# wsakobe/CylinderTag

Measured on AMD Instinct MI355X. Metric: frames/sec detect() 1920x1080, higher is better.
Workload: dtype u8; 1 GPU; synthetic 1920x1080 random-stripe frames, 4096 per step over 1 GPU(s), 4 planted CTag_2f12c markers each, detect(img,5,true,5), inputs resident in HBM; frames_per_gpu=4096, chunk=4096, parallelism=frames sharded, dp1, gather=none (1 GPU)

## Files before the change

cylindertag_amd/csrc/k_quad.hip:

```cpp
#include "ctag_internal.h"
#include "ctag_math.h"
#include <cstdio>
#include <type_traits>
#include <cstdlib>

namespace ctag {

struct QuadPtrs {
    const uint16_t* labels;
    const int32_t* tile_base;
    const int32_t* root_of;
    const int32_t* ncand;
    const Candidate* cand;
    QuadOut* quads;
    uint32_t* frame_flags;
    int32_t* line_count;
    int32_t* clp_used;
    uint32_t* cl_pool;
    LineDesc* line_desc;
    int32_t* line_sorted;
    int32_t* line_long;
    float* line_fit;
    CandAux* cand_aux;
    const uint8_t* pick_table;
// ... 38 lines not shown
__device__ __forceinline__ bool solve2x2(float a00, float a01, float a10, float a11, float b0, float b1, float& x0, float& x1) {
    double d = (double)a00 * a11 - (double)a01 * a10;
    if (d == 0.) return false;
    d = 1. / d;
    const float t = (float)(((double)b0 * a11 - (double)b1 * a01) * d);
    x1 = (float)(((double)b1 * a00 - (double)b0 * a10) * d);
    x0 = t;
    return true;
}

struct CvRng {
    uint64_t state;
    __device__ unsigned next() {
        state = (uint64_t)(unsigned)state * 4164903690U + (unsigned)(state >> 32);
        return (unsigned)state;
    }
};

#ifndef CTAG_WCAP
#define CTAG_WCAP 16
#endif
#ifndef CTAG_WUNROLL
#define CTAG_WUNROLL 2
#endif
#define CTAG_PRAGMA_(x) _Pragma(#x)
#define CTAG_PRAGMA(x) CTAG_PRAGMA_(x)
constexpr int kWCap = CTAG_WCAP;
struct GlobalPts {
    const uint32_t* p;
    __device__ __forceinline__ float2 operator()(int j) const {
        const uint32_t v = p[j];
        return make_float2((float)ux(v), (float)uy(v));
    }
};
struct LdsPts {
    const float2* p;
    __device__ __forceinline__ float2 operator()(int j) const { return p[j]; }
};
struct LdsPackedPts {
    const uint32_t* p;
    __device__ __forceinline__ float2 operator()(int j) const {
        const uint32_t v = p[j];
        return make_float2((float)ux(v), (float)uy(v));
    }
};
struct TablePicks {
    const uint8_t* t;
    __device__ __forceinline__ int operator()(int i) const { return t[i]; }
};
struct ListPicks {
    const uint16_t* t;
    __device__ __forceinline__ int operator()(int i) const { return t[i]; }
};
struct AllPicks {
    __device__ __forceinline__ int operator()(int i) const { return i; }
};
struct RestartResult {
    float line[4];
    double err;
};
__device__ __forceinline__ RestartResult restart_result(const float* res, int rstride) {
    RestartResult r;
    for (int q = 0; q < 4; q++) r.line[q] = res[q * rstride];
    const uint64_t lo = ctm::f32_to_bits(res[4 * rstride]), hi = ctm::f32_to_bits(res[5 * rstride]);
    r.err = ctm::bits_to_f64(lo | (hi << 32));
    return r;
}
template <class Pts, class Picks>
__device__ __forceinline__ void welsch_first_fit(const Pts pts, const Picks picks, int npick, float* line) {
    double x = 0, y = 0, x2 = 0, y2 = 0, xy = 0, w = 0;
    for (int i = 0; i < npick; i++) {
        const float2 p = pts(picks(i));
        const float px = p.x, py = p.y;
        x += px;
        y += py;
        x2 += px * px;
        y2 += py * py;
        xy += px * py;
        w += 1.f;
    }
    moments_to_line(x, y, x2, y2, xy, w, line);
}
template <int WS, class Pts>
__device__ __forceinline__ bool welsch_rounds(const Pts pts, int n, double EPS, float* line, double& err, int it0, int it_stop, bool resume, float* wc, int ncache) {
    float prev[4] = {0.f, 0.f, 0.f, 0.f};
    const float c = 1 / 2.9846f;
#ifdef CTAG_WELSCH_MINERR_IN_LOOP
    double berr = 1.7976931348623157e308;
    float bl[4] = {0.f, 0.f, 0.f, 0.f};
#define CTAG_WELSCH_HAND_ON()       \
    do {                            \
        for (int q = 0; q < 4; q++) line[q] = bl[q]; \
        err = berr;                 \
    } while (0)
#else
#define CTAG_WELSCH_HAND_ON() do { } while (0)
#endif
    for (int it = it0; it < 30; it++) {
        if (it > 0 && !(resume && it == it0)) {
            const float t = line[0] * prev[0] + line[1] * prev[1];
            if (t >= ctm::kAcosBelowTenMilli) {
                const float dx = ctm::fabs32(line[2] - prev[2]);
                const float dy = ctm::fabs32(line[3] - prev[3]);
                const float d = dx > dy ? dx : dy;
                if (d < 0.01f) {
                    CTAG_WELSCH_HAND_ON();
                    return true;
                }
            }
        }
        if (it == it_stop) return false;
        const float lx = line[2], ly = line[3], nx = line[1], ny = -line[0];
        double sum_w = 0;
        err = 0;
        float2 pn0 = pts(min(0, n - 1));
        CTAG_PRAGMA(unroll CTAG_WUNROLL)
        for (int j = 0; j < ncache; j++) {
            const float2 p = pn0;
            pn0 = pts(j + 1);
            const float x = p.x - lx, y = p.y - ly;
            const float r = ctm::fabs32(nx * x + ny * y);
            err += r;
            const float wj = ctm::exp32_nonpos(-r * r * c * c);
            wc[j * WS] = wj;
            sum_w += wj;
        }
        float2 pn1 = pts(min(ncache, n - 1));
        CTAG_PRAGMA(unroll CTAG_WUNROLL)
        for (int j = ncache; j < n; j++) {
            const float2 p = pn1;
            pn1 = pts(j + 1);
            const float x = p.x - lx, y = p.y - ly;
            const float r = ctm::fabs32(nx * x + ny * y);
            err += r;
            sum_w += ctm::exp32_nonpos(-r * r * c * c);
        }
#ifdef CTAG_WELSCH_MINERR_IN_LOOP
        if (err < berr) {
            berr = err;
            for (int q = 0; q < 4; q++) bl[q] = line[q];
            if (err < EPS) return true;
        }
#else
        if (err < EPS) return true;
#endif
        double x = 0, y = 0, x2 = 0, y2 = 0, xy = 0, w = 0;
        if (ctm::fabs64(sum_w) > 1.1920928955078125e-07) {
            const double inv = 1. / sum_w;
            float2 pn2 = pts(min(0, n - 1));
            CTAG_PRAGMA(unroll CTAG_WUNROLL)
            for (int j = 0; j < ncache; j++) {
                const float2 p = pn2;
                pn2 = pts(j + 1);
                const float px = p.x, py = p.y;
                const float wj = (float)(wc[j * WS] * inv);
                x += wj * px;
                y += wj * py;
                x2 += wj * px * px;
                y2 += wj * py * py;
                xy += wj * px * py;
                w += wj;
            }
            float2 pn3 = pts(min(ncache, n - 1));
            CTAG_PRAGMA(unroll CTAG_WUNROLL)
            for (int j = ncache; j < n; j++) {
                const float2 p = pn3;
                pn3 = pts(j + 1);
                const float px = p.x, py = p.y;
                const float r = ctm::fabs32(nx * (px - lx) + ny * (py - ly));
                const float wj = (float)(ctm::exp32_nonpos(-r * r * c * c) * inv);
                x += wj * px;
                y += wj * py;
                x2 += wj * px * px;
                y2 += wj * py * py;
                xy += wj * px * py;
                w += wj;
            }
        } else {
            float2 pn4 = pts(min(0, n - 1));
            for (int j = 0; j < n; j++) {
                const float2 p = pn4;
                pn4 = pts(j + 1);
                const float px = p.x, py = p.y;
                x += px;
                y += py;
                x2 += px * px;
                y2 += py * py;
                xy += px * py;
                w += 1.f;
            }
        }
        prev[0] = line[0];
        prev[1] = line[1];
        prev[2] = line[2];
        prev[3] = line[3];
        moments_to_line(x, y, x2, y2, xy, w, line);
    }
    CTAG_WELSCH_HAND_ON();
    return true;
}
#undef CTAG_WELSCH_HAND_ON
__device__ __forceinline__ void restart_store(float* res, int rstride, const float* line, double err) {
    for (int q = 0; q < 4; q++) res[q * rstride] = line[q];
    const uint64_t eb = ctm::f64_to_bits(err);
    res[4 * rstride] = ctm::bits_to_f32((uint32_t)eb);
    res[5 * rstride] = ctm::bits_to_f32((uint32_t)(eb >> 32));
}
template <int WS, class Pts, class Picks>
__device__ __forceinline__ void welsch_restart(const Pts pts, int n, const Picks picks, int npick, double EPS, float* res, int rstride, float* wc) {
    float line[4];
    double err = 0;
    welsch_first_fit(pts, picks, npick, line);
    (void)welsch_rounds<WS>(pts, n, EPS, line, err, 0, 30, false, wc, min(n, kWCap));
    restart_store(res, rstride, line, err);
}

#ifndef CTAG_PACK_WORDS
#define CTAG_PACK_WORDS 5120
#endif
#ifndef CTAG_PACK_WAVES
#define CTAG_PACK_WAVES 2
#endif
constexpr int kPackWords = CTAG_PACK_WORDS;
#ifndef CTAG_PACK_WAVES_P2
#define CTAG_PACK_WAVES_P2 4
#endif
constexpr int kPackWordsSmall = 2560, kPackWavesSmall = 4, kPackWavesSmallP2 = CTAG_PACK_WAVES_P2;
constexpr int kUnwind = 8;
constexpr int kWaveWords = 8192;
constexpr int kWaveWordsMax = 36864;
__host__ __device__ __forceinline__ int pack_points(int w, int h) { return min(2 * (w + h), w * h) + 1; }
__host__ __device__ __forceinline__ int pack_need(int w, int h) {
    const int C = pack_points(w, h);
    return ((w + 1) & ~1) + 2 * h + 2 * C + 4;
}
constexpr int kScanWords = 2048;
__host__ __device__ __forceinline__ int scan_need(int w, int h) { return w + 3 * h + 4; }
constexpr int kMaskScanWords = 512, kMaskScanWordsLarge = 2048;
// ... 1520 lines not shown
                else
                    sg_expand_line<SG>(W, n, init, end, sl, lane0, sgshift, k_thr_expand, (float)(g.hcols > g.hrows ? g.hcols : g.hrows), REFPRM ? 3.0e-6f : P.expand_eps, nl, nr);
                rdp_mark(2);
                const int m = end - init + 1 + nl + nr;
                const int a = ((init - nl) % n + n) % n;
                const int b = (end + nr) % n;
                const bool wrap = a > b;
                const int span0 = wrap ? n - 1 : b;
                const int keep = tri2(span0) <= k_c2_near ? 1 : 0;
                const int offc = cl_off[cnt_b];
                for (int k = sl; k < m; k += SG) {
                    int idx;
                    if (!wrap) {
                        idx = b - k;
                    } else {
                        idx = (k < n - a) ? (n - 1 - k) : (b - (k - (n - a)));
                    }
                    if (offc + k < C + 64) CLg[offc + k] = W[idx];
                }
                const int new_n = n - m + keep;
                if (!wrap) {
                    for (int k = sl; k < new_n; k += SG) {
                        int src;
                        if (k < a) src = k;
                        else if (keep && k == a) src = b;
                        else src = k - keep + m;
                        Wn[k] = W[src];
                    }
                } else {
                    const int mid = a - b - 1;
                    for (int k = sl; k < new_n; k += SG) Wn[k] = (k < mid) ? W[b + 1 + k] : W[n - 1];
                }
                SG_SYNC();
                const int back = wrap ? 0 : a;
                cl_off[cnt_b + 1] = min(offc + m, C + 64);
                cnt_b++;
                init = (back >= new_n) ? 0 : back;
                n = new_n;
                uint32_t* t = W;
                W = Wn;
                Wn = t;
                rdp_mark(3);
                break;
            }
        }
        if (SG == 64 && P.stamps && lane == 0)
        {
            for (int q = 0; q < 4; q++) atomicAdd(&P.stamps[16 + q], rdp_acc[q]);
            for (int q = 0; q < 3; q++) atomicAdd(&P.stamps[20 + q], exp_dbg[q]);
        }
        stamp(3);
        bool ok = true;
        for (int j = 0; j < 4; j++) {
            const int len = (j < cnt_b) ? (cl_off[j + 1] - cl_off[j]) : 0;
            if (len < 2) ok = false;
        }
        if (cl_off[min(cnt_b, 4)] >= C + 64) ok = false;
        int l0 = -1;
        if (ok) {
            if (sl == 0) l0 = atomicAdd(&P.line_count[frame], 4);
            l0 = __shfl(l0, lane0);
            if (l0 + 4 > P.line_cap) {
                ok = false;
                if (sl == 0) atomicOr(&P.frame_flags[frame], CTAG_FLAG_POOL_OVERFLOW);
            }
        }
        if (ok && sl < 4) {
            LineDesc d;
            d.off = (uint32_t)(p0 + cl_off[sl]);
            d.n = cl_off[sl + 1] - cl_off[sl];
            P.line_desc[(size_t)frame * P.line_cap + l0 + sl] = d;
        }
        if (sl == 0) {
            aux->line0 = ok ? l0 : -1;
            aux->acx = ok ? acx : 0.f;
            aux->acy = ok ? acy : 0.f;
            aux->n_boundary = n_boundary;
        }
        stamp(4);
    }
}

constexpr int kWShort = 10;
constexpr int kLineSortThreads = 1024;
__global__ __launch_bounds__(kLineSortThreads) void k_line_sort(QuadPtrs P, int nframes) {
    __shared__ int s_n[kLdsLines];
    __shared__ int s_long;
    const int frame = blockIdx.x;
    if (frame >= nframes) return;
    const int L = min(P.line_count[frame], P.line_cap);
    const LineDesc* d = P.line_desc + (size_t)frame * P.line_cap;
    int32_t* out = P.line_sorted + (size_t)frame * P.line_cap;
    if (threadIdx.x == 0) s_long = 0;
    __syncthreads();
    if (L > kLdsLines) {
        constexpr int kB = 2048;
        static_assert(kB - 1 > kLatPoints && kB + 1 <= kLdsLines, "shared bucket");
        auto bucket_of = [&](int n) { return kB - 1 - min(n, kB - 1); };
        for (int b = threadIdx.x; b <= kB; b += kLineSortThreads) s_n[b] = 0;
        __syncthreads();
        int mine = 0;
        for (int i = threadIdx.x; i < L; i += kLineSortThreads) {
            const int n = d[i].n;
            atomicAdd(&s_n[bucket_of(n)], 1);
            mine += n > kWShort ? 1 : 0;
        }
        if (mine) atomicAdd(&s_long, mine);
        __syncthreads();
        if (threadIdx.x == 0) {
            P.line_long[frame] = s_long;
            int run = 0;
            for (int b = 0; b < kB; b++) {
                const int v = s_n[b];
                s_n[b] = run;
                run += v;
            }
        }
        __syncthreads();
        for (int i = threadIdx.x; i < L; i += kLineSortThreads) out[atomicAdd(&s_n[bucket_of(d[i].n)], 1)] = i;
        return;
    }
    int mine = 0;
    for (int i = threadIdx.x; i < L; i += kLineSortThreads) {
        const int n = d[i].n;
        s_n[i] = n;
        mine += n > kWShort ? 1 : 0;
    }
    if (mine) atomicAdd(&s_long, mine);
    __syncthreads();
    if (threadIdx.x == 0) P.line_long[frame] = s_long;
    for (int i = threadIdx.x; i < L; i += kLineSortThreads) {
        const int ni = s_n[i];
        int rank = 0;
        for (int j = 0; j < L; j++) {
            const int nj = s_n[j];
            rank += (nj > ni || (nj == ni && j < i)) ? 1 : 0;
        }
        out[rank] = i;
    }
}

__device__ __forceinline__ void welsch_select(const QuadPtrs& P, int frame, int lid, int n, const float* res, int kstride, int rstride, int count) {
    const double EPS = n * 1.1920928955078125e-07;
    double min_err = 1.7976931348623157e308;
    float best[4] = {0.f, 0.f, 0.f, 0.f};
    for (int kk = 0; kk < count; kk++) {
        const RestartResult r = restart_result(res + kk * kstride, rstride);
        if (r.err < min_err) {
            min_err = r.err;
            for (int q = 0; q < 4; q++) best[q] = r.line[q];
#ifndef CTAG_WELSCH_MINERR_IN_LOOP
            if (r.err < EPS) break;
#endif
        }
    }
    float* o = P.line_fit + ((size_t)frame * P.line_cap + lid) * 4;
    for (int q = 0; q < 4; q++) o[q] = best[q];
}

#ifndef CTAG_WELSCH_BLOCK_WAVES
#define CTAG_WELSCH_BLOCK_WAVES 4
#endif
constexpr int kWB = CTAG_WELSCH_BLOCK_WAVES;
constexpr int kWT = kWB * 64;
constexpr int kWE = kWT / 20;
constexpr int kWRes = 10;
#ifdef CTAG_WELSCH_MINERR_IN_LOOP
#undef CTAG_WELSCH_REGROUP_AT
#define CTAG_WELSCH_REGROUP_AT 30
#endif
#ifndef CTAG_WELSCH_REGROUP_AT
#define CTAG_WELSCH_REGROUP_AT 2
#endif
constexpr int kWRegroupAt = CTAG_WELSCH_REGROUP_AT;
#ifndef CTAG_WPTS
#define CTAG_WPTS 128
#endif
constexpr int kWPts = CTAG_WPTS;
#ifndef CTAG_WPTSU
#define CTAG_WPTSU 240
#endif
constexpr int kWPtsU = CTAG_WPTSU;
static_assert(kWPtsU % 2 == 0 && kWPtsU < kPickN, "packed rows: an odd number of words, picks from the byte table");
static_assert(kWE * 20 <= kWT && kWCap >= kWRes + 6 && kWRes >= 5 && kWRes >= kWShort && kWPts < kPickN && kWE * kWPts * 8 >= kWT * 10 * 2 && (kWPts + 1) % 32 == 1, "k_welsch LDS layout");
struct WelschLds {
    float wc[kWCap * kWT];
    union {
    uint32_t ptu[kWE][kWPtsU + 1];
    float2 pt[kWE][kWPts + 1];
    };
    const uint32_t* gpts[kWE];
    int n[kWE];
    int lid[kWE];
    int cnt[kWB];
};

template <int MODE>
__device__ __forceinline__ void welsch_block_run(const QuadPtrs& P, WelschLds& S, int frame) {
    const int tid = threadIdx.x, lane = tid & 63, wave = tid >> 6;
    constexpr bool STAGED = MODE != 2;
    using PtsT = typename std::conditional<MODE == 0, LdsPts, typename std::conditional<MODE == 1, LdsPackedPts, GlobalPts>::type>::type;
    auto pts_of = [&](int e) -> PtsT {
        if constexpr (MODE == 0) return LdsPts{S.pt[e]};
        else if constexpr (MODE == 1) return LdsPackedPts{S.ptu[e]};
        else return GlobalPts{S.gpts[e]};
    };
    float line[4] = {0.f, 0.f, 0.f, 0.f};
    double err = 0;
    bool fin = true;
    int item = tid;
    for (int phase = 0; phase < 2; phase++) {
        bool run;
        if (phase == 0) {
            run = tid < kWE * 20 && S.n[min(tid / 20, kWE - 1)] > 0;
            if (P.stamps) {
                const unsigned long long act = __ballot(run);
                if (lane == 0) atomicAdd(&P.stamps[24], (unsigned long long)__popcll(act));
            }
        } else {
            const unsigned long long bal = __ballot(!fin);
            if (lane == 0) S.cnt[wave] = __popcll(bal);
            __syncthreads();
            int base = 0, total = 0;
#pragma unroll
            for (int w = 0; w < kWB; w++) {
                const int c = S.cnt[w];
                base += w < wave ? c : 0;
                total += c;
            }
            if (!fin) {
                const int r = base + __popcll(bal & ((1ull << lane) - 1ull));
#pragma unroll
                for (int q = 0; q < 4; q++) S.wc[q * kWT + r] = line[q];
                S.wc[4 * kWT + r] = __int_as_float(tid);
            }
            __syncthreads();
            if (P.stamps && tid == 0) {
                atomicAdd(&P.stamps[25], (unsigned long long)total);
                atomicAdd(&P.stamps[26], 1ull);
            }
            run = tid < total;
            if (run) {
#pragma unroll
                for (int q = 0; q < 4; q++) line[q] = S.wc[q * kWT + tid];
                item = __float_as_int(S.wc[4 * kWT + tid]);
            }
        }
        if (run) {
            const int e = item / 20, k = item - e * 20;
            const int n = S.n[e];
            const double EPS = n * 1.1920928955078125e-07;
            const PtsT pts = pts_of(e);
            if (phase == 0) {
                if (STAGED || n < kPickN) {
                    welsch_first_fit(pts, TablePicks{P.pick_table + ((size_t)n * 20 + k) * 10}, min(n, 10), line);
                } else if (n < kPickN2) {
                    welsch_first_fit(pts, ListPicks{P.pick_table16 + ((size_t)(n - kPickN) * 20 + k) * 10}, 10, line);
                } else {
                    uint16_t* pk = reinterpret_cast<uint16_t*>(&S.pt[0][0]) + tid * 10;
                    CvRng rng;
                    rng.state = 0xffffffffffffffffULL;
                    for (int kk = 0; kk <= k; kk++) {
                        int got = 0;
                        while (got < 10) {
                            const int j = (int)(rng.next() % (unsigned)n);
                            bool dup = false;
                            for (int q = 0; q < got; q++) dup |= (pk[q] == j);
                            if (!dup) pk[got++] = (uint16_t)j;
                        }
                    }
                    for (int a = 1; a < 10; a++) {
                        const uint16_t v = pk[a];
                        int b = a - 1;
                        while (b >= 0 && pk[b] > v) {
                            pk[b + 1] = pk[b];
                            b--;
                        }
                        pk[b + 1] = v;
                    }
                    welsch_first_fit(pts, ListPicks{pk}, 10, line);
                }
            }
            fin = welsch_rounds<kWT>(pts, n, EPS, line, err, phase == 0 ? 0 : kWRegroupAt, phase == 0 ? kWRegroupAt : 30, phase != 0, S.wc + tid, min(n, phase == 0 ? kWCap : kWRes));
            if (fin) restart_store(S.wc + kWRes * kWT + item, kWT, line, err);
        } else {
            fin = true;
        }
    }
    __syncthreads();
    if (tid < kWE && S.n[tid] > 0) welsch_select(P, frame, S.lid[tid], S.n[tid], S.wc + kWRes * kWT + tid * 20, 1, kWT, 20);
}

__device__ __forceinline__ void welsch_block(const QuadPtrs& P, WelschLds& S, int frame, int first, int L) {
    const int tid = threadIdx.x;
    if (tid < kWE) {
        int n = 0, lid = 0;
        const uint32_t* p = nullptr;
        if (first + tid < L) {
            lid = P.line_sorted[(size_t)frame * P.line_cap + first + tid];
            const LineDesc d = P.line_desc[(size_t)frame * P.line_cap + lid];
            n = d.n;
            p = P.cl_pool + (size_t)frame * P.cl_cap + d.off;
        }
        S.n[tid] = n;
        S.lid[tid] = lid;
        S.gpts[tid] = p;
    }
    __syncthreads();
    const int n0 = S.n[0];
    if (n0 <= kWPts) {
        for (int idx = tid; idx < kWE * kWPts; idx += kWT) {
            const int e = idx / kWPts, j = idx - e * kWPts;
            if (j < S.n[e]) {
                const uint32_t v = S.gpts[e][j];
                S.pt[e][j] = make_float2((float)ux(v), (float)uy(v));
            }
        }
        __syncthreads();
        welsch_block_run<0>(P, S, frame);
    } else if (n0 <= kWPtsU) {
        for (int idx = tid; idx < kWE * kWPtsU; idx += kWT) {
            const int e = idx / kWPtsU, j = idx - e * kWPtsU;
            if (j < S.n[e]) S.ptu[e][j] = S.gpts[e][j];
        }
        __syncthreads();
        welsch_block_run<1>(P, S, frame);
    } else {
        welsch_block_run<2>(P, S, frame);
    }
}

__device__ __forceinline__ void welsch_short(const QuadPtrs& P, WelschLds& S, int frame, int first, int L) {
    const int tid = threadIdx.x;
    if (first + tid >= L) return;
    const int lid = P.line_sorted[(size_t)frame * P.line_cap + first + tid];
    const LineDesc d = P.line_desc[(size_t)frame * P.line_cap + lid];
    const int n = d.n;
    welsch_restart<kWT>(GlobalPts{P.cl_pool + (size_t)frame * P.cl_cap + d.off}, n, AllPicks{}, n, n * 1.1920928955078125e-07, S.wc + tid, kWT, S.wc + tid);
    welsch_select(P, frame, lid, n, S.wc + tid, 0, kWT, 1);
}

__device__ __forceinline__ bool welsch_lat_takes(const QuadPtrs& P, int frame, int L) {
    if (L > kLatLines) return false;
    if (L == 0) return true;
    const int longest = P.line_sorted[(size_t)frame * P.line_cap];
    return P.line_desc[(size_t)frame * P.line_cap + longest].n <= kLatPoints;
}

__device__ __forceinline__ double ordered_sum(double a, const float* src, int n) {
    int j = 0;
    for (; j + 8 <= n; j += 8) {
        float v[8];
#pragma unroll
        for (int u = 0; u < 8; u++) v[u] = src[j + u];
#pragma unroll
        for (int u = 0; u < 8; u++) a += v[u];
    }
    for (; j < n; j++) a += src[j];
    return a;
}

constexpr int kLatChunk = 128;
static_assert(kLatPoints % kLatChunk == 0 && kLatChunk % 64 == 0, "k_welsch_lat: register / chunk layout");
#ifndef CTAG_WLAT_WAVES
#define CTAG_WLAT_WAVES 5
#endif
__global__ __launch_bounds__(64) __attribute__((amdgpu_waves_per_eu(CTAG_WLAT_WAVES))) void k_welsch_lat(QuadPtrs P, int nframes, float* rs) {
    constexpr int NQ = kLatPoints / 64, CQ = kLatChunk / 64, NC = kLatPoints / kLatChunk;
    __shared__ float s_r[kLatChunk], s_w[kLatChunk];
    __shared__ float s_t[6][kLatChunk];
    __shared__ double s_sum[8];
    __shared__ uint16_t s_pk[10];
    const int frame = blockIdx.z, k = blockIdx.x, lane = threadIdx.x;
    if (frame >= nframes) return;
    const int L = min(P.line_count[frame], P.line_cap);
    if (!welsch_lat_takes(P, frame, L)) return;
    const float c = 1 / 2.9846f;
    for (int rank = blockIdx.y; rank < L; rank += gridDim.y) {
        const unsigned long long dbg_t0 = P.stamps ? __builtin_amdgcn_s_memtime() : 0ull;
        __syncthreads();
        const int lid = P.line_sorted[(size_t)frame * P.line_cap + rank];
        const LineDesc d = P.line_desc[(size_t)frame * P.line_cap + lid];
        const int n = d.n;
        const uint32_t* pts = P.cl_pool + (size_t)frame * P.cl_cap + d.off;
        uint32_t pp[NQ];
        float ww[NQ];
#pragma unroll
        for (int q = 0; q < NQ; q++) {
            pp[q] = pts[min(lane + 64 * q, n - 1)];
            ww[q] = 0.f;
        }
        const int npick = min(n, 10);
        if (lane == 0) {
            if (n < kPickN) {
                const uint8_t* t = P.pick_table + ((size_t)n * 20 + k) * 10;
                for (int q = 0; q < npick; q++) s_pk[q] = t[q];
            } else if (n < kPickN2) {
                const uint16_t* t = P.pick_table16 + ((size_t)(n - kPickN) * 20 + k) * 10;
                for (int q = 0; q < npick; q++) s_pk[q] = t[q];
            } else {
                CvRng rng;
                rng.state = 0xffffffffffffffffULL;
                for (int kk = 0; kk <= k; kk++) {
                    int got = 0;
                    while (got < npick) {
                        const int j = (int)(rng.next() % (unsigned)n);
                        bool dup = false;
                        for (int q = 0; q < got; q++) dup |= (s_pk[q] == j);
                        if (!dup) s_pk[got++] = (uint16_t)j;
                    }
                }
                for (int a = 1; a < npick; a++) {
                    const uint16_t v = s_pk[a];
                    int b = a - 1;
                    while (b >= 0 && s_pk[b] > v) {
                        s_pk[b + 1] = s_pk[b];
                        b--;
                    }
                    s_pk[b + 1] = v;
                }
            }
        }
// ... 61 lines not shown
            }
#else
            if (err < EPS) break;
#endif
            const bool weighted = ctm::fabs64(sum_w) > 1.1920928955078125e-07;
            const double inv = weighted ? 1. / sum_w : 0.;
            acc = 0;
#pragma unroll
            for (int ch = 0; ch < NC; ch++) {
                if (ch * kLatChunk >= n) break;
                if (ch > 0) __syncthreads();
#pragma unroll
                for (int u = 0; u < CQ; u++) {
                    const int q = ch * CQ + u, j = 64 * u + lane;
                    const float fx = (float)ux(pp[q]), fy = (float)uy(pp[q]);
                    if (weighted) {
                        const float wj = (float)(ww[q] * inv);
                        s_t[0][j] = wj * fx;
                        s_t[1][j] = wj * fy;
                        s_t[2][j] = wj * fx * fx;
                        s_t[3][j] = wj * fy * fy;
                        s_t[4][j] = wj * fx * fy;
                        s_t[5][j] = wj;
                    } else {
                        s_t[0][j] = fx;
                        s_t[1][j] = fy;
                        s_t[2][j] = fx * fx;
                        s_t[3][j] = fy * fy;
                        s_t[4][j] = fx * fy;
                        s_t[5][j] = 1.f;
                    }
                }
                __syncthreads();
                if (lane < 6) acc = ordered_sum(acc, s_t[lane], min(kLatChunk, n - ch * kLatChunk));
            }
            if (lane < 6) s_sum[2 + lane] = acc;
            __syncthreads();
            prev[0] = line[0];
            prev[1] = line[1];
            prev[2] = line[2];
            prev[3] = line[3];
            moments_to_line(s_sum[2], s_sum[3], s_sum[4], s_sum[5], s_sum[6], s_sum[7], line);
        }
#ifdef CTAG_WELSCH_MINERR_IN_LOOP
        for (int q = 0; q < 4; q++) line[q] = bl[q];
        err = berr;
#endif
        if (lane == 0) {
            float* o = rs + (((size_t)frame * kLatLines + rank) * 20 + k) * 6;
            o[0] = line[0];
            o[1] = line[1];
            o[2] = line[2];
            o[3] = line[3];
            *reinterpret_cast<double*>(o + 4) = err;
            if (P.stamps && rank < 8 && (k == 0 || k == 19)) P.stamps[16 + 8 + (k ? 1 : 0) * 4 + (rank >> 1)] = __builtin_amdgcn_s_memtime() - dbg_t0;
        }
    }
}

__device__ __forceinline__ void welsch_pick(const QuadPtrs& P, int frame, int rank, const float* rs) {
    const int lid = P.line_sorted[(size_t)frame * P.line_cap + rank];
    const int n = P.line_desc[(size_t)frame * P.line_cap + lid].n;
    const double EPS = n * 1.1920928955078125e-07;
    double min_err = 1.7976931348623157e308;
    float best[4] = {0.f, 0.f, 0.f, 0.f};
    const float* r = rs + ((size_t)frame * kLatLines + rank) * 20 * 6;
    for (int kk = 0; kk < 20; kk++) {
        const double e = *reinterpret_cast<const double*>(r + kk * 6 + 4);
        if (e < min_err) {
            min_err = e;
            for (int q = 0; q < 4; q++) best[q] = r[kk * 6 + q];
#ifndef CTAG_WELSCH_MINERR_IN_LOOP
            if (e < EPS) break;
#endif
        }
    }
    float* o = P.line_fit + ((size_t)frame * P.line_cap + lid) * 4;
    for (int q = 0; q < 4; q++) o[q] = best[q];
}

#ifndef CTAG_WELSCH_PRIO_RANKS
#define CTAG_WELSCH_PRIO_RANKS 3
#endif
#ifndef CTAG_WELSCH_WAVES
#define CTAG_WELSCH_WAVES 5
#endif
__global__ __launch_bounds__(kWT) __attribute__((amdgpu_waves_per_eu(CTAG_WELSCH_WAVES, CTAG_WELSCH_WAVES))) void k_welsch(QuadPtrs P, int nframes, const float* lat_rs, int gy_long) {
    const int frame = blockIdx.x;
    if (frame >= nframes) return;
    const int L = min(P.line_count[frame], P.line_cap);
    if (lat_rs && welsch_lat_takes(P, frame, L)) {
        for (int rank = (int)blockIdx.y * kWT + (int)threadIdx.x; rank < L; rank += (int)gridDim.y * kWT) welsch_pick(P, frame, rank, lat_rs);
        return;
    }
    if (blockIdx.y < (unsigned)CTAG_WELSCH_PRIO_RANKS) __builtin_amdgcn_s_setprio(3);
    __shared__ WelschLds S;
    const int nlong = min(P.line_long[frame], L);
    if ((int)blockIdx.y < gy_long) {
        for (int first = (int)blockIdx.y * kWE; first < nlong; first += gy_long * kWE) {
            welsch_block(P, S, frame, first, nlong);
            __syncthreads();
        }
    } else {
        for (int first = nlong + ((int)blockIdx.y - gy_long) * kWT; first < L; first += ((int)gridDim.y - gy_long) * kWT) welsch_short(P, S, frame, first, L);
    }
}

template <int LANES>
__device__ __forceinline__ void quad_final_one(const QuadPtrs& P, const FrameGeom& g, int frame, int ci, int sub);
template <int LANES>
__global__ __launch_bounds__(64) void k_quad_final(QuadPtrs P, FrameGeom g, int nframes) {
    const int frame = blockIdx.y;
    if (frame >= nframes) return;
    const int nc = min(P.ncand[frame], P.cand_cap);
    constexpr int PER = 64 / LANES;
    for (int ci = (int)((blockIdx.x + frame) % gridDim.x) * PER + (int)threadIdx.x / LANES; ci < nc; ci += (int)gridDim.x * PER)
        quad_final_one<LANES>(P, g, frame, ci, (int)threadIdx.x % LANES);
}
template <int LANES>
__device__ __forceinline__ void quad_final_one(const QuadPtrs& P, const FrameGeom& g, int frame, int ci, int sub) {
    const CandAux aux = P.cand_aux[(size_t)frame * P.cand_cap + ci];
    QuadOut* out = P.quads + (size_t)frame * P.cand_cap + ci;
    if (sub == 0) out->n_boundary = aux.n_boundary;
    if (aux.line0 < 0) {
        if (sub == 0) out->valid = 0;
        return;
    }
    const int areaPx = P.cand[(size_t)frame * P.cand_cap + ci].area;
    const float acx = aux.acx, acy = aux.acy;
    float lf[4][4];
    {
        const float* src = P.line_fit + ((size_t)frame * P.line_cap + aux.line0) * 4;
        for (int j = 0; j < 4; j++)
            for (int q = 0; q < 4; q++) lf[j][q] = src[j * 4 + q];
    }
    CornerPre raw[6];
    bool ok6[6];
    {
        int q = 0;
#pragma unroll
        for (int j = 0; j < 3; j++)
#pragma unroll
            for (int k = j + 1; k < 4; k++) {
                const float a00 = lf[j][1], a01 = -lf[j][0], a10 = lf[k][1], a11 = -lf[k][0];
                const float b0 = lf[j][1] * lf[j][2] - lf[j][0] * lf[j][3];
                const float b1 = lf[k][1] * lf[k][2] - lf[k][0] * lf[k][3];
                CornerPre c{0.f, 0.f, 0.f, 0.f};
                bool ok = false;
                if (LANES == 1 || sub == q) {
                    ok = solve2x2(a00, a01, a10, a11, b0, b1, c.x, c.y);
                    if (ok) {
                        c.dis = ctm::sqrt32((c.x - acx) * (c.x - acx) + (c.y - acy) * (c.y - acy));
                        c.ang = (float)(ctm::atan2_32(c.y - acy, c.x - acx) * 180 / 3.1415926535897932384626433832795);
                        ok = c.dis < g.hcols && c.dis < g.hrows;
                    }
                }
                raw[q] = c;
                ok6[q] = ok;
                q++;
            }
        if constexpr (LANES > 1) {
            const int l0 = (int)threadIdx.x & ~(LANES - 1);
#pragma unroll
            for (int u = 0; u < 6; u++) {
                raw[u].x = __shfl(raw[u].x, l0 + u);
                raw[u].y = __shfl(raw[u].y, l0 + u);
                raw[u].dis = __shfl(raw[u].dis, l0 + u);
                raw[u].ang = __shfl(raw[u].ang, l0 + u);
                ok6[u] = __shfl((int)ok6[u], l0 + u) != 0;
// ... 100 lines not shown
    } else if (pl.prescan) {
        if (pl.mask_scan)
            if (pl.small_cfg) hipLaunchKernelGGL((k_silhouette_mask<4, 32, kMaskScanWords>), dim3(nframes, pl.mscan_gx), dim3(64), 0, s, P, g, nframes);
            else hipLaunchKernelGGL((k_silhouette_mask<8, 64, kMaskScanWordsLarge>), dim3(nframes, 2 * pl.mscan_gx), dim3(64), 0, s, P, g, nframes);
        else
            hipLaunchKernelGGL((k_quad_edges_packed<64, kScanWords, CTAG_SCAN_WAVES, false, true, 3>), dim3(nframes, pl.scan_gx), dim3(64), 0, s, P, g, nframes, 0);
        if (pl.small_cfg) {
            hipLaunchKernelGGL((k_quad_edges_packed<8, kPackWordsSmall, kPackWavesSmall, false, REF, 1, true>), grid, dim3(64), 0, s, P, g, nframes, 0);
            hipLaunchKernelGGL((k_quad_edges_packed<8, kPackWordsSmall, kPackWavesSmallP2, false, REF, 2>), grid, dim3(64), 0, s, P, g, nframes, 0);
        } else {
            hipLaunchKernelGGL((k_quad_edges_packed<8, kPackWords, CTAG_PACK_WAVES, false, REF, 0, true>), grid, dim3(64), 0, s, P, g, nframes, 0);
        }
    } else if (pl.small_cfg) {
        hipLaunchKernelGGL((k_quad_edges_packed<8, kPackWordsSmall, kPackWavesSmall, false, REF, 1>), grid, dim3(64), 0, s, P, g, nframes, 0);
        hipLaunchKernelGGL((k_quad_edges_packed<8, kPackWordsSmall, kPackWavesSmallP2, false, REF, 2>), grid, dim3(64), 0, s, P, g, nframes, 0);
    } else {
        hipLaunchKernelGGL((k_quad_edges_packed<8, kPackWords, CTAG_PACK_WAVES, false, REF>), grid, dim3(64), 0, s, P, g, nframes, 0);
    }
    if (mid) (void)hipEventRecord(mid, s);
    int dev = 0;
    (void)hipGetDevice(&dev);
    dev = dev < 0 || dev >= 64 ? 0 : dev;
    static bool have[64] = {false};
    if (!have[dev]) {
        (void)hipFuncSetAttribute(reinterpret_cast<const void*>(&k_quad_edges_packed<64, kWaveWordsMax, 1, true, REF>), hipFuncAttributeMaxDynamicSharedMemorySize,
                                  kWaveWordsMax * 4);
        have[dev] = true;
    }
    hipLaunchKernelGGL((k_quad_edges_packed<64, kWaveWords, 1, false, REF>), dim3(nframes, pl.big_cols), dim3(64), 0, sb, P, g, nframes, 0);
    hipLaunchKernelGGL((k_quad_edges_packed<64, kWaveWordsMax, 1, true, REF>), dim3(nframes, pl.big_max_gx), dim3(64), kWaveWordsMax * 4, s_max, P, g, nframes, kWaveWords);
}

hipError_t launch_quads(const ChunkPlan& pl, const Workspace& ws, hipStream_t s, hipEvent_t* ev5) {
    const int nframes = pl.nframes;
    int evi = 0;
    auto mark = [&]() {
        if (ev5) (void)hipEventRecord(ev5[evi++], s);
    };
    QuadPtrs P{ws.labels, ws.tile_base, ws.root_of, ws.ncand, ws.cand, ws.quads, ws.frame_flags,
               ws.line_count, ws.clp_used, ws.cl_pool, ws.line_desc, ws.line_sorted, ws.line_long, ws.line_fit, ws.cand_aux, ws.pick_table, ws.pick_table16, ws.pool_tile, ws.member_head, ws.member_next, ws.npacks, ws.packs, ws.pack_order, nullptr, ws.kp.thr_line, ws.kp.thr_expand, ws.kp.rac, ws.kp.c2_far, ws.kp.c2_near,
               ws.cand_cap, ws.line_cap, ws.cl_cap, ws.kp.expand_eps};
    static unsigned long long* d_stamps = nullptr;
    if (pl.quad_stamps) {
        if (!d_stamps) (void)hipMalloc(reinterpret_cast<void**>(&d_stamps), 32 * 8);
        (void)hipMemsetAsync(d_stamps, 0, 32 * 8, s);
        P.stamps = d_stamps;
    }
    P.mask = pl.fused ? reinterpret_cast<const uint64_t*>(ws.half) : nullptr;
    P.mask_words = ws.g.hcols >> 6;
    const int pack_words = pl.small_cfg ? kPackWordsSmall : kPackWords;
    const int scan_words = pl.mask_scan ? -(pl.small_cfg ? kMaskScanWords : kMaskScanWordsLarge) : pl.prescan ? kScanWords : 0;
    hipLaunchKernelGGL(k_pack, dim3(nframes), dim3(pl.latency ? 1024 : 64), 0, s, P, nframes, pl.pack_max, pl.big_points, pack_words, scan_words);
    mark();
    const bool fork = pl.fork && ws.aux_stream != nullptr;
    hipStream_t sb = s;
    if (fork) {
        (void)hipEventRecord(ws.ev_fork, s);
        (void)hipStreamWaitEvent(ws.aux_stream, ws.ev_fork, 0);
        sb = ws.aux_stream;
    }
    (pl.refprm ? launch_quad_edges<true> : launch_quad_edges<false>)(pl, P, ws.g, s, sb, fork ? s : sb, ev5 ? ev5[evi++] : nullptr);
    if (fork) {
        (void)hipEventRecord(ws.ev_join, sb);
        (void)hipStreamWaitEvent(s, ws.ev_join, 0);
    }
    mark();
    hipLaunchKernelGGL(k_line_sort, dim3(nframes), dim3(kLineSortThreads), 0, s, P, nframes);
    mark();
    const bool welsch_lat = pl.latency && ws.welsch_rs;
    if (welsch_lat) {
        hipLaunchKernelGGL(k_welsch_lat, dim3(20, 512, nframes), dim3(64), 0, s, P, nframes, ws.welsch_rs);
    }
    hipLaunchKernelGGL(k_welsch, dim3(nframes, pl.welsch_gx + pl.welsch_gs), dim3(kWT), 0, s, P, nframes, welsch_lat ? ws.welsch_rs : (const float*)nullptr, pl.welsch_gx);
    mark();
    if (pl.latency) hipLaunchKernelGGL(k_quad_final<8>, dim3(std::min(ws.cand_cap, kLdsCand) / 8, nframes), dim3(64), 0, s, P, ws.g, nframes);
    else hipLaunchKernelGGL(k_quad_final<1>, dim3(std::min(ws.cand_cap, kLdsCand) / 64, nframes), dim3(64), 0, s, P, ws.g, nframes);
    if (pl.quad_stamps) {
        unsigned long long h[32];
        (void)hipStreamSynchronize(s);
        (void)hipMemcpy(h, d_stamps, sizeof(h), hipMemcpyDeviceToHost);
        if (h[16] | h[17] | h[18] | h[19])
            fprintf(stderr, "[whole-wave rdp ticks] corner scan %llu split rounds %llu expand_line %llu clusters + erase %llu\n", h[16], h[17], h[18], h[19]),
            fprintf(stderr, "[whole-wave expand_line] initial sums %llu ticks, %llu rounds, %llu of them through the exact fits\n", h[20], h[21], h[22]);
        if (h[26]) fprintf(stderr, "[k_welsch] %llu restarts in %llu blocks, %llu (%.1f %%) went on after the regroup at iteration %d\n", h[24], h[26], h[25], 100.0 * h[25] / (h[24] ? h[24] : 1), kWRegroupAt);
        else if (h[24]) fprintf(stderr, "[k_welsch_lat ticks] restart 0 of the edges of rank 0 / 2 / 4 / 6: %llu %llu %llu %llu; restart 19: %llu %llu %llu %llu\n", h[24], h[25], h[26], h[27], h[28], h[29], h[30], h[31]);
        for (int b = 0; b < 16; b += 8) {
            unsigned long long tot = 0;
            h[b + 0] += h[b + 7];
            for (int i = 0; i < 5; i++) tot += h[b + i];
            if (!tot) continue;
            fprintf(stderr, "[%s] row scan %llu of the silhouette phase's %llu ticks\n", b ? "whole-wave" : "packed", h[b + 7], h[b + 0]);
            fprintf(stderr, "[%s cycles] header %.1f%% keys+init %.1f%% | silhouette %.1f%% traversal %.1f%% centroid/rotate %.1f%% rdp %.1f%% export %.1f%% (total %llu)\n",
                    b ? "whole-wave" : "packed", 100.0 * h[b + 6] / (tot + h[b + 5] + h[b + 6]), 100.0 * h[b + 5] / (tot + h[b + 5] + h[b + 6]), 100.0 * h[b + 0] / tot,
                    100.0 * h[b + 1] / tot, 100.0 * h[b + 2] / tot, 100.0 * h[b + 3] / tot, 100.0 * h[b + 4] / tot, tot);
        }
    }
    return hipGetLastError();
}

void build_pick_table(uint8_t* table, uint16_t* table16) {
    for (int n = 0; n < kPickN2; n++) {
        uint64_t state = 0xffffffffffffffffULL;
        for (int k = 0; k < 20; k++) {
            uint16_t pk[10] = {0, 0, 0, 0, 0, 0, 0, 0, 0, 0};
            if (n >= 2) {
                const int npick = n < 10 ? n : 10;
                int got = 0;
                while (got < npick) {
                    state = (uint64_t)(unsigned)state * 4164903690U + (unsigned)(state >> 32);
                    const int j = (int)((unsigned)state % (unsigned)n);
                    bool dup = false;
                    for (int q = 0; q < got; q++) dup |= (pk[q] == j);
                    if (!dup) pk[got++] = (uint16_t)j;
                }
                for (int a = 1; a < npick; a++) {
                    const uint16_t v = pk[a];
                    int b = a - 1;
                    while (b >= 0 && pk[b] > v) {
                        pk[b + 1] = pk[b];
                        b--;
                    }
                    pk[b + 1] = v;
                }
            }
            for (int q = 0; q < 10; q++) {
                if (n < kPickN) table[((size_t)n * 20 + k) * 10 + q] = (uint8_t)pk[q];
                else table16[((size_t)(n - kPickN) * 20 + k) * 10 + q] = pk[q];
            }
        }
    }
}

}
```

Baseline: 252,600 frames/s.

## Carve Welsch LDS per block size and let survivors borrow idle lanes' weight columns

```diff
diff --git a/cylindertag_amd/csrc/k_quad.hip b/cylindertag_amd/csrc/k_quad.hip
--- a/cylindertag_amd/csrc/k_quad.hip
+++ b/cylindertag_amd/csrc/k_quad.hip
@@ -144,7 +144,8 @@
     moments_to_line(x, y, x2, y2, xy, w, line);
 }
 template <int WS, class Pts>
-__device__ __forceinline__ bool welsch_rounds(const Pts pts, int n, double EPS, float* line, double& err, int it0, int it_stop, bool resume, float* wc, int ncache) {
+__device__ __forceinline__ bool welsch_rounds(const Pts pts, int n, double EPS, float* line, double& err, int it0, int it_stop, bool resume, float* wc, int ncache,
+                                              int csplit = 0x7fffffff, int coff = 0, unsigned long long* stamps = nullptr) {
     float prev[4] = {0.f, 0.f, 0.f, 0.f};
     const float c = 1 / 2.9846f;
 #ifdef CTAG_WELSCH_MINERR_IN_LOOP
@@ -184,7 +185,7 @@
             const float r = ctm::fabs32(nx * x + ny * y);
             err += r;
             const float wj = ctm::exp32_nonpos(-r * r * c * c);
-            wc[j * WS] = wj;
+            wc[j * WS + (j >= csplit ? coff : 0)] = wj;
             sum_w += wj;
         }
         float2 pn1 = pts(min(ncache, n - 1));
@@ -209,13 +210,17 @@
         double x = 0, y = 0, x2 = 0, y2 = 0, xy = 0, w = 0;
         if (ctm::fabs64(sum_w) > 1.1920928955078125e-07) {
             const double inv = 1. / sum_w;
+            if (stamps) {
+                atomicAdd(&stamps[0], (unsigned long long)ncache);
+                atomicAdd(&stamps[1], (unsigned long long)(n - ncache));
+            }
             float2 pn2 = pts(min(0, n - 1));
             CTAG_PRAGMA(unroll CTAG_WUNROLL)
             for (int j = 0; j < ncache; j++) {
                 const float2 p = pn2;
                 pn2 = pts(j + 1);
                 const float px = p.x, py = p.y;
-                const float wj = (float)(wc[j * WS] * inv);
+                const float wj = (float)(wc[j * WS + (j >= csplit ? coff : 0)] * inv);
                 x += wj * px;
                 y += wj * py;
                 x2 += wj * px * px;
@@ -1902,6 +1907,7 @@
 }
 
 constexpr int kWShort = 10;
+constexpr int kLineSortExact = 2047;
 constexpr int kLineSortThreads = 1024;
 __global__ __launch_bounds__(kLineSortThreads) void k_line_sort(QuadPtrs P, int nframes) {
     __shared__ int s_n[kLdsLines];
@@ -1915,7 +1921,7 @@
     __syncthreads();
     if (L > kLdsLines) {
         constexpr int kB = 2048;
-        static_assert(kB - 1 > kLatPoints && kB + 1 <= kLdsLines, "shared bucket");
+        static_assert(kB - 1 > kLatPoints && kB + 1 <= kLdsLines && kB - 1 == kLineSortExact, "shared bucket");
         auto bucket_of = [&](int n) { return kB - 1 - min(n, kB - 1); };
         for (int b = threadIdx.x; b <= kB; b += kLineSortThreads) s_n[b] = 0;
         __syncthreads();
@@ -1984,7 +1990,6 @@
 constexpr int kWB = CTAG_WELSCH_BLOCK_WAVES;
 constexpr int kWT = kWB * 64;
 constexpr int kWE = kWT / 20;
-constexpr int kWRes = 10;
 #ifdef CTAG_WELSCH_MINERR_IN_LOOP
 #undef CTAG_WELSCH_REGROUP_AT
 #define CTAG_WELSCH_REGROUP_AT 30
@@ -2002,29 +2007,58 @@
 #endif
 constexpr int kWPtsU = CTAG_WPTSU;
 static_assert(kWPtsU % 2 == 0 && kWPtsU < kPickN, "packed rows: an odd number of words, picks from the byte table");
-static_assert(kWE * 20 <= kWT && kWCap >= kWRes + 6 && kWRes >= 5 && kWRes >= kWShort && kWPts < kPickN && kWE * kWPts * 8 >= kWT * 10 * 2 && (kWPts + 1) % 32 == 1, "k_welsch LDS layout");
-struct WelschLds {
-    float wc[kWCap * kWT];
-    union {
-    uint32_t ptu[kWE][kWPtsU + 1];
-    float2 pt[kWE][kWPts + 1];
-    };
+#ifndef CTAG_WELSCH_WAVES
+#define CTAG_WELSCH_WAVES 5
+#endif
+#ifndef CTAG_WELSCH_LDS
+#define CTAG_WELSCH_LDS (CTAG_WELSCH_WAVES >= 5 ? 32768 : 40960)
+#endif
+constexpr int kWLdsBytes = CTAG_WELSCH_LDS;
+constexpr int kWTabBytes = kWE * (8 + 4 + 4) + kWB * 4;
+constexpr int kWWords = (kWLdsBytes - kWTabBytes) / 4;
+constexpr int kWResRows = 6;
+#ifndef CTAG_WELSCH_TWO_COLUMNS_MAX
+#define CTAG_WELSCH_TWO_COLUMNS_MAX (kWT / 2)
+#endif
+constexpr int kWTwoMax = CTAG_WELSCH_TWO_COLUMNS_MAX;
+static_assert(kWTwoMax >= 0 && kWTwoMax <= kWT / 2, "k_welsch: a survivor borrows the column of a lane without work");
+__host__ __device__ constexpr int welsch_pitch(int n0) { return (n0 + 1) | 1; }
+constexpr int kWPickFrom = kPickN2 < kLineSortExact ? kPickN2 : kLineSortExact;
+__host__ __device__ constexpr int welsch_point_bytes(int n0) {
+    return n0 <= kWPts ? kWE * welsch_pitch(n0) * 8 : n0 <= kWPtsU ? kWE * welsch_pitch(n0) * 4 : n0 >= kWPickFrom ? kWT * 10 * 2 : 0;
+}
+__host__ __device__ constexpr int welsch_rows(int n0) { return (kWWords * 4 - welsch_point_bytes(n0)) / (kWT * 4); }
+constexpr int kWRowsMin = welsch_rows(kWPts) < welsch_rows(kWPtsU) ? (welsch_rows(kWPts) < welsch_rows(kWPickFrom) ? welsch_rows(kWPts) : welsch_rows(kWPickFrom))
+                                                                    : (welsch_rows(kWPtsU) < welsch_rows(kWPickFrom) ? welsch_rows(kWPtsU) : welsch_rows(kWPickFrom));
+static_assert(kWE * 20 <= kWT && kWPts < kPickN && kWPtsU < kPickN && kWPtsU < kLineSortExact, "k_welsch: 20 lanes per edge, staged edges pick from the tables");
+static_assert(kWRowsMin - kWResRows >= kWShort && kWRowsMin - kWResRows >= 5, "k_welsch: the least carve holds the results above kWShort cached rows and the regroup's five state rows");
+static_assert(kWWords >= (kWShort > kWResRows ? kWShort : kWResRows) * kWT, "welsch_short: kWShort weight rows (and its result) at the array's base");
+static_assert(welsch_rows(kWPickFrom) * kWT * 4 + kWT * 10 * 2 <= kWWords * 4, "k_welsch: the replayed pick lists fit the point area");
+static_assert(kWTabBytes % 8 == 0 && kWLdsBytes % 8 == 0, "k_welsch: the tables keep the array's alignment");
+struct alignas(16) WelschLds {
+    uint32_t a[kWWords];
     const uint32_t* gpts[kWE];
     int n[kWE];
     int lid[kWE];
     int cnt[kWB];
+    __device__ __forceinline__ float* wc() { return reinterpret_cast<float*>(a); }
 };
+static_assert(sizeof(WelschLds) == kWLdsBytes, "k_welsch LDS budget");
 
 template <int MODE>
-__device__ __forceinline__ void welsch_block_run(const QuadPtrs& P, WelschLds& S, int frame) {
+__device__ __forceinline__ void welsch_block_run(const QuadPtrs& P, WelschLds& S, int frame, int rows, int pitch) {
     const int tid = threadIdx.x, lane = tid & 63, wave = tid >> 6;
     constexpr bool STAGED = MODE != 2;
     using PtsT = typename std::conditional<MODE == 0, LdsPts, typename std::conditional<MODE == 1, LdsPackedPts, GlobalPts>::type>::type;
+    float* const wc = S.wc();
+    uint32_t* const area = S.a + rows * kWT;
+    const int crows = rows - kWResRows;
     auto pts_of = [&](int e) -> PtsT {
-        if constexpr (MODE == 0) return LdsPts{S.pt[e]};
-        else if constexpr (MODE == 1) return LdsPackedPts{S.ptu[e]};
+        if constexpr (MODE == 0) return LdsPts{reinterpret_cast<const float2*>(area) + e * pitch};
+        else if constexpr (MODE == 1) return LdsPackedPts{area + e * pitch};
         else return GlobalPts{S.gpts[e]};
     };
+    int cap = rows, csplit = rows, coff = 0;
     float line[4] = {0.f, 0.f, 0.f, 0.f};
     double err = 0;
     bool fin = true;
@@ -2051,19 +2085,24 @@
             if (!fin) {
                 const int r = base + __popcll(bal & ((1ull << lane) - 1ull));
 #pragma unroll
-                for (int q = 0; q < 4; q++) S.wc[q * kWT + r] = line[q];
-                S.wc[4 * kWT + r] = __int_as_float(tid);
+                for (int q = 0; q < 4; q++) wc[q * kWT + r] = line[q];
+                wc[4 * kWT + r] = __int_as_float(tid);
             }
             __syncthreads();
+            const bool two = total <= kWTwoMax;
+            cap = two ? 2 * crows : crows;
+            csplit = crows;
+            coff = kWT / 2 - crows * kWT;
             if (P.stamps && tid == 0) {
                 atomicAdd(&P.stamps[25], (unsigned long long)total);
                 atomicAdd(&P.stamps[26], 1ull);
+                if (total > 0) atomicAdd(&P.stamps[two ? 30 : 29], 1ull);
             }
             run = tid < total;
             if (run) {
 #pragma unroll
-                for (int q = 0; q < 4; q++) line[q] = S.wc[q * kWT + tid];
-                item = __float_as_int(S.wc[4 * kWT + tid]);
+                for (int q = 0; q < 4; q++) line[q] = wc[q * kWT + tid];
+                item = __float_as_int(wc[4 * kWT + tid]);
             }
         }
         if (run) {
@@ -2077,7 +2116,7 @@
                 } else if (n < kPickN2) {
                     welsch_first_fit(pts, ListPicks{P.pick_table16 + ((size_t)(n - kPickN) * 20 + k) * 10}, 10, line);
                 } else {
-                    uint16_t* pk = reinterpret_cast<uint16_t*>(&S.pt[0][0]) + tid * 10;
+                    uint16_t* pk = reinterpret_cast<uint16_t*>(area) + tid * 10;
                     CvRng rng;
                     rng.state = 0xffffffffffffffffULL;
                     for (int kk = 0; kk <= k; kk++) {
@@ -2101,14 +2140,15 @@
                     welsch_first_fit(pts, ListPicks{pk}, 10, line);
                 }
             }
-            fin = welsch_rounds<kWT>(pts, n, EPS, line, err, phase == 0 ? 0 : kWRegroupAt, phase == 0 ? kWRegroupAt : 30, phase != 0, S.wc + tid, min(n, phase == 0 ? kWCap : kWRes));
-            if (fin) restart_store(S.wc + kWRes * kWT + item, kWT, line, err);
+            fin = welsch_rounds<kWT>(pts, n, EPS, line, err, phase == 0 ? 0 : kWRegroupAt, phase == 0 ? kWRegroupAt : 30, phase != 0, wc + tid, min(n, cap), csplit, coff,
+                                     P.stamps ? P.stamps + 27 : nullptr);
+            if (fin) restart_store(wc + crows * kWT + item, kWT, line, err);
         } else {
             fin = true;
         }
     }
     __syncthreads();
-    if (tid < kWE && S.n[tid] > 0) welsch_select(P, frame, S.lid[tid], S.n[tid], S.wc + kWRes * kWT + tid * 20, 1, kWT, 20);
+    if (tid < kWE && S.n[tid] > 0) welsch_select(P, frame, S.lid[tid], S.n[tid], wc + crows * kWT + tid * 20, 1, kWT, 20);
 }
 
 __device__ __forceinline__ void welsch_block(const QuadPtrs& P, WelschLds& S, int frame, int first, int L) {
@@ -2128,25 +2168,27 @@
     }
     __syncthreads();
     const int n0 = S.n[0];
+    const int pitch = welsch_pitch(n0), rows = welsch_rows(n0);
+    uint32_t* const area = S.a + rows * kWT;
+    const int e = tid / 20, j0 = tid - e * 20;
     if (n0 <= kWPts) {
-        for (int idx = tid; idx < kWE * kWPts; idx += kWT) {
-            const int e = idx / kWPts, j = idx - e * kWPts;
-            if (j < S.n[e]) {
+        if (e < kWE) {
+            float2* const row = reinterpret_cast<float2*>(area) + e * pitch;
+            for (int j = j0; j < S.n[e]; j += 20) {
                 const uint32_t v = S.gpts[e][j];
-                S.pt[e][j] = make_float2((float)ux(v), (float)uy(v));
+                row[j] = make_float2((float)ux(v), (float)uy(v));
             }
         }
         __syncthreads();
-        welsch_block_run<0>(P, S, frame);
+        welsch_block_run<0>(P, S, frame, rows, pitch);
     } else if (n0 <= kWPtsU) {
-        for (int idx = tid; idx < kWE * kWPtsU; idx += kWT) {
-            const int e = idx / kWPtsU, j = idx - e * kWPtsU;
-            if (j < S.n[e]) S.ptu[e][j] = S.gpts[e][j];
+        if (e < kWE) {
+            for (int j = j0; j < S.n[e]; j += 20) area[e * pitch + j] = S.gpts[e][j];
         }
         __syncthreads();
-        welsch_block_run<1>(P, S, frame);
+        welsch_block_run<1>(P, S, frame, rows, pitch);
     } else {
-        welsch_block_run<2>(P, S, frame);
+        welsch_block_run<2>(P, S, frame, rows, pitch);
     }
 }
 
@@ -2156,8 +2198,8 @@
     const int lid = P.line_sorted[(size_t)frame * P.line_cap + first + tid];
     const LineDesc d = P.line_desc[(size_t)frame * P.line_cap + lid];
     const int n = d.n;
-    welsch_restart<kWT>(GlobalPts{P.cl_pool + (size_t)frame * P.cl_cap + d.off}, n, AllPicks{}, n, n * 1.1920928955078125e-07, S.wc + tid, kWT, S.wc + tid);
-    welsch_select(P, frame, lid, n, S.wc + tid, 0, kWT, 1);
+    welsch_restart<kWT>(GlobalPts{P.cl_pool + (size_t)frame * P.cl_cap + d.off}, n, AllPicks{}, n, n * 1.1920928955078125e-07, S.wc() + tid, kWT, S.wc() + tid);
+    welsch_select(P, frame, lid, n, S.wc() + tid, 0, kWT, 1);
 }
 
 __device__ __forceinline__ bool welsch_lat_takes(const QuadPtrs& P, int frame, int L) {
@@ -2385,9 +2427,6 @@
 #ifndef CTAG_WELSCH_PRIO_RANKS
 #define CTAG_WELSCH_PRIO_RANKS 3
 #endif
-#ifndef CTAG_WELSCH_WAVES
-#define CTAG_WELSCH_WAVES 5
-#endif
 __global__ __launch_bounds__(kWT) __attribute__((amdgpu_waves_per_eu(CTAG_WELSCH_WAVES, CTAG_WELSCH_WAVES))) void k_welsch(QuadPtrs P, int nframes, const float* lat_rs, int gy_long) {
     const int frame = blockIdx.x;
     if (frame >= nframes) return;
@@ -2654,7 +2693,11 @@
         if (h[16] | h[17] | h[18] | h[19])
             fprintf(stderr, "[whole-wave rdp ticks] corner scan %llu split rounds %llu expand_line %llu clusters + erase %llu\n", h[16], h[17], h[18], h[19]),
             fprintf(stderr, "[whole-wave expand_line] initial sums %llu ticks, %llu rounds, %llu of them through the exact fits\n", h[20], h[21], h[22]);
-        if (h[26]) fprintf(stderr, "[k_welsch] %llu restarts in %llu blocks, %llu (%.1f %%) went on after the regroup at iteration %d\n", h[24], h[26], h[25], 100.0 * h[25] / (h[24] ? h[24] : 1), kWRegroupAt);
+        if (h[26]) {
+            fprintf(stderr, "[k_welsch] %llu restarts in %llu blocks, %llu (%.1f %%) went on after the regroup at iteration %d\n", h[24], h[26], h[25], 100.0 * h[25] / (h[24] ? h[24] : 1), kWRegroupAt);
+            fprintf(stderr, "[k_welsch cache] second-pass points: %llu cached, %llu recomputed (%.1f %%); blocks after the regroup: %llu one column, %llu two columns\n", h[27], h[28],
+                    100.0 * h[28] / (h[27] + h[28] ? h[27] + h[28] : 1), h[29], h[30]);
+        }
         else if (h[24]) fprintf(stderr, "[k_welsch_lat ticks] restart 0 of the edges of rank 0 / 2 / 4 / 6: %llu %llu %llu %llu; restart 19: %llu %llu %llu %llu\n", h[24], h[25], h[26], h[27], h[28], h[29], h[30], h[31]);
         for (int b = 0; b < 16; b += 8) {
             unsigned long long tot = 0;
```

Measured after the change: 252,500 frames/s. Within noise of the previous version (-0.0%).
